# lisqzqng/GaVA-CLIP

Hardware: AMD Instinct MI355X
Metric: clips/sec (8-frame 224^2 ViT-B/16 VitaCLIP.forward) (higher is better)
Workload: dtype fp16; 1 GPU; c2: ViT-B/16, 8 frames, 224^2, batch 64/GPU, 3 classes; clips_per_gpu=64, global_batch=64, frames=8, classes=3, weights=random-init, parallelism=single GPU, text_tower=split-precision GEMMs (3 MFMA passes), fp32 softmax core

## Files before the change

gava_clip_amd/csrc/forward.hip:

```cpp
#include "common.h"
#include "internal.h"
#include <stdlib.h>
#include <mutex>

namespace {

struct SideStream {
  hipStream_t s = nullptr;
  hipEvent_t fork[64], join[64];
  bool ok = false, tried = false;
  bool get() {
    if (tried) return ok;
    tried = true;
    const char* e = getenv("GAVA_SIDE_STREAM");
    if (e && e[0] == '0') return false;
    int lo = 0, hi = 0;
    if (hipDeviceGetStreamPriorityRange(&lo, &hi) != hipSuccess) return false;
    if (hipStreamCreateWithPriority(&s, hipStreamNonBlocking, hi) != hipSuccess) return false;
    for (int i = 0; i < 64; ++i)
      if (hipEventCreateWithFlags(&fork[i], hipEventDisableTiming) != hipSuccess ||
          hipEventCreateWithFlags(&join[i], hipEventDisableTiming) != hipSuccess) return false;
    ok = true;
    return true;
  }
};

struct Fc1Probe {
  hipEvent_t ev[64][2];
  bool made = false;
  int on = 0;
  int n = 0;
  unsigned long long valid = 0;
  bool ensure() {
    if (made) return true;
    for (int i = 0; i < 64; ++i)
      for (int k = 0; k < 2; ++k)
        if (hipEventCreate(&ev[i][k]) != hipSuccess) return false;
    made = true;
    return true;
  }
};

constexpr int MAX_DEVICES = 64;
struct DeviceCtx {
  std::mutex mu;
  SideStream side;
  Fc1Probe probe;
};
DeviceCtx g_dev[MAX_DEVICES];
DeviceCtx& device_ctx() {
  int d = 0;
  if (hipGetDevice(&d) != hipSuccess || d < 0) d = 0;
  return g_dev[d % MAX_DEVICES];
}

struct Side {
  const SideStream& st; hipStream_t s; bool two;
  Side(SideStream& side, hipStream_t s, int layers) : st(side), s(s), two(side.get() && layers <= 64) {}
  gava_stream_t stream() const { return two ? (gava_stream_t)st.s : (gava_stream_t)s; }
  int fork(int i) const {
    return !two || (hipEventRecord(st.fork[i], s) == hipSuccess && hipStreamWaitEvent(st.s, st.fork[i], 0) == hipSuccess)
               ? GAVA_OK : GAVA_ELAUNCH;
  }
  int done(int i) const { return !two || hipEventRecord(st.join[i], st.s) == hipSuccess ? GAVA_OK : GAVA_ELAUNCH; }
  int join(int i) const { return !two || hipStreamWaitEvent(s, st.join[i], 0) == hipSuccess ? GAVA_OK : GAVA_ELAUNCH; }
  int cus(bool ln1_folded) const { return two ? (ln1_folded ? 32 : 8) : 0; }
};

struct Carver {
  char* base; size_t off, cap;
  Carver(void* b, size_t c) : base((char*)b), off(0), cap(c) {}
  void* take(size_t bytes) {
    const size_t a = (off + 255) & ~(size_t)255;
    off = a + bytes;
    return base ? (void*)(base + a) : nullptr;
  }
};

#define TRY(x)              \
  do {                      \
    const int _e = (x);     \
    if (_e != GAVA_OK) return _e; \
  } while (0)

int ln(const float* in, long in_stride, const int32_t* idx, const float* g, const float* b, void* o16, long o16s,
       float* o32, long o32s, int rows, int D, int prec, gava_stream_t s, int split = 0, const float* g2 = nullptr,
       const float* b2 = nullptr, void* ohi = nullptr, void* olo = nullptr, long ohls = 0) {
  gava_layernorm_args a{};
  a.gamma2 = g2; a.beta2 = b2;
  a.out_hi = ohi; a.out_lo = olo; a.out_hl_stride = ohls;
  a.in = in; a.in_stride = in_stride; a.in_row_index = idx; a.gamma = g; a.beta = b;
  a.out16 = o16; a.out16_stride = o16s; a.out32 = o32; a.out32_stride = o32s;
  a.rows = rows; a.D = D; a.prec = prec; a.split_out = split;
  return gava_layernorm(&a, s);
}

struct Fold {
  void* x16 = nullptr; long ld_x16 = 0; float* rowsum = nullptr; int reduced = 0;
  const float* stats = nullptr; const float* s = nullptr; const float* t = nullptr;
  const float* partials = nullptr;
  const void* r16 = nullptr; const void* rlo = nullptr; void* xlo = nullptr;
};

struct Lo8 {
  const void* A8 = nullptr; const void* W8 = nullptr; int exp = 0;
  void* out8 = nullptr; long ldo8 = 0; void* x8 = nullptr; long ldx8 = 0;
};

int gemm_x(int w_lo, const void* A, long lda, const void* W, long ldw, const float* bias, void* out, long ldo, int M, int N, int K,
           int epi, int prec, gava_stream_t s, const float* resid = nullptr, long ldr = 0, int scale_cols = 0,
           float scale = 1.f, int split_out = 0, void* aux_out = nullptr, const Fold* fold = nullptr, int cu_reserve = 0,
           const Lo8* l8 = nullptr) {
  gava_gemm_args a{};
  a.w_lo = w_lo ? 1 : 0;
  if (w_lo) ldw *= 2;
  if (l8) {
    if (l8->W8) {
      a.w_lo = 2; a.A8 = l8->A8; a.lda8 = 2 * lda; a.W8 = l8->W8; a.ldw8 = 2 * ldw; a.w8_exp = l8->exp;
    }
    a.out8 = l8->out8; a.ldo8 = l8->ldo8; a.x8_out = l8->x8; a.ld_x8 = l8->ldx8;
// ... 70 lines not shown
  w.XNC = c.take(BT * 3 * D * 2);
  w.QC = c.take(BT * D * 2);
  w.MIXC = c.take(BT * 3 * D * 2);
  w.HIDC = c.take(BT * 3 * F * 2);
  {
    const long per_slot = R * (D / 64) * 8, reduced = (R + 255) / 256 * 256 * 4 * 8 + 1024;
    w.RSUM = (float*)c.take(per_slot > reduced ? per_slot : reduced);
  }
  w.STATS = (float*)c.take((R + 255) / 256 * 256 * 8);
  w.Xn8 = m->w_lo == 2 ? c.take((size_t)R * 2 * D) : nullptr;
  w.HID8 = m->w_lo == 2 ? c.take((size_t)R * 2 * F) : nullptr;
  w.total = (c.off + 255) & ~(size_t)255;
  return w;
}

int check_vision(const gava_vision_model* m) {
  if (!m || !m->layer) return GAVA_EINVAL;
  if (m->B <= 0 || m->T_in <= 0 || m->T_model <= 0 || m->layers <= 0) return GAVA_EINVAL;
  if (m->size % m->P || m->D != m->H * 64 || m->D % 128 || m->F % 128 || m->E % 128) return GAVA_EINVAL;
  if (m->D > 1024) return GAVA_EINVAL;
  if (((long)m->B * m->T_in) % m->T_model) return GAVA_EINVAL;
  return GAVA_OK;
}

bool fused_stats(long R, int D) { return R >= 8192 && D % 256 == 0 && D <= 1024 && D >= 256; }

bool pair_stream(const gava_vision_model* m) {
  const long g = m->size / m->P, R = (long)m->B * m->T_in * (g * g + 1);
  const int D = m->D, F = m->F, WL = m->w_lo ? 2 : 1;
  bool pair = m->w_lo != 2 && m->layers >= 2 && fused_stats(R, D) &&
              gava::gemm_takes_pair((int)R, D, D, D, (long)WL * D) && gava::gemm_takes_pair((int)R, D, F, F, (long)WL * F);
  for (int i = 0; pair && i + 1 < m->layers; ++i) pair = m->layer[i].w_fc1_fold && m->layer[i + 1].w_qkv_fold;
  return pair;
}


struct VisionShape {
  int n, BT, R, D, F, E, H, G, Tm, pr, Kp, SR;
  long fs;
  explicit VisionShape(const gava_vision_model* m)
      : n((m->size / m->P) * (m->size / m->P)), BT(m->B * m->T_in), R(BT * (n + 1)), D(m->D), F(m->F), E(m->E), H(m->H),
        G(m->G), Tm(m->T_model), pr(m->prec), Kp(patch_k(m)), SR(G + 2 * BT), fs((long)(n + 1) * D) {}
};

int open_vision(const gava_vision_model* m, const float* x, const float* cls_x, const float* summary, void* workspace,
                size_t workspace_bytes, VisionWs* w) {
  TRY(check_vision(m));
  if ((!x && !m->clips) || !cls_x || !summary || !workspace) return GAVA_EINVAL;
  *w = carve_vision(m, workspace, workspace_bytes);
  return w->total > workspace_bytes ? GAVA_EWORKSPACE : GAVA_OK;
}

int embed(const gava_vision_model* m, const VisionShape& v, const float* x, int wl, float* out, void* scratch,
          gava_stream_t stream) {
  gava_gemm_args a{};
  a.W = m->w_patch; a.ldw = (wl ? 2 : 1) * v.Kp; a.bias = m->b_patch; a.w_lo = wl;
  a.out = out; a.ldo = v.D; a.M = v.BT * v.n; a.N = v.D; a.K = v.Kp; a.epilogue = GAVA_EPI_F32_PATCH; a.prec = v.pr;
  a.pos = m->pos_embed; a.time = m->time_embed; a.n_patches = v.n; a.T = m->T_in;
  TRY(patch_operand(m, x, scratch, stream, &a));
  TRY(gava_gemm(&a, stream));
  return gava::cls_embed(out, m->cls_token, m->pos_embed, m->time_embed, v.BT, m->T_in, v.D, v.fs, (hipStream_t)stream);
}

int prompt_path(const VisionShape& v, const gava_vision_layer& L, int wl, const VisionWs& w, const float* X, const void* hi,
                void* skv, gava_stream_t ss) {
  const int D = v.D, BT = v.BT, pr = v.pr;
  if (hi) {
    TRY(gemm_x(wl, hi, v.fs, L.w_cls, D, L.b_cls, w.CP, D, BT, D, D, GAVA_EPI_F32, pr, ss));
  } else {
    TRY(ln(X, v.fs, nullptr, nullptr, nullptr, w.CLS16, D, nullptr, 0, BT, D, pr, ss));
    TRY(gemm_x(wl, w.CLS16, D, L.w_cls, D, L.b_cls, w.CP, D, BT, D, D, GAVA_EPI_F32, pr, ss));
  }
  TRY(ln(w.CP, D, nullptr, L.sln_g, L.sln_b, w.CPn, D, nullptr, 0, BT, D, pr, ss));
  TRY(gemm_x(wl, w.CPn, D, L.w_sqkv, D, L.b_sqkv, w.SQKV, 3 * D, BT, 3 * D, D, GAVA_EPI_H16, pr, ss, nullptr, 0, D, 0.125f));
  {
    gava_attention_args a{};
    const unsigned short* q = (const unsigned short*)w.SQKV;
    a.q = q; a.k = q + D; a.v = q + 2 * D; a.ld_qkv = 3 * D; a.out = w.SMIX; a.ld_out = D;
    a.batch = BT / v.Tm; a.heads = v.H; a.n_q = v.Tm; a.n_kmain = v.Tm; a.prec = pr;
    TRY(gava_attention(&a, ss));
  }
  TRY(gemm_x(wl, w.SMIX, D, L.w_sout, D, L.b_sout, w.SUMM, D, BT, D, D, GAVA_EPI_F32, pr, ss, w.CP, D));
  TRY(gava::side_ln(L.global_prompts, L.local_prompts, w.CP, w.SUMM, L.ln1_g, L.ln1_b, w.SIDEn, v.G, v.Tm, BT, D, pr, (hipStream_t)ss));
  const unsigned short* wkv = (const unsigned short*)L.w_qkv + (long)D * (wl ? 2 : 1) * D;
  return gemm_x(wl, w.SIDEn, D, wkv, D, L.b_qkv + D, skv, 2 * D, v.SR, 2 * D, D, GAVA_EPI_H16, pr, ss);
}

struct FoldPlan {
  const VisionWs& w; int R, D; bool fused;
  FoldPlan(const VisionWs& w, int R, int D) : w(w), R(R), D(D), fused(fused_stats(R, D)) {}
  Fold produce() const {
    Fold p; p.x16 = w.Xn; p.ld_x16 = D; p.rowsum = w.RSUM; p.reduced = fused ? 1 : 0;
    return p;
  }
  Fold consume(const float* s, const float* t) const {
    Fold c; c.s = s; c.t = t;
    if (fused) c.partials = w.RSUM; else c.stats = w.STATS;
    return c;
  }
  int stats(gava_stream_t stream) const { return fused ? GAVA_OK : gava_row_stats(w.RSUM, D / 64, D, R, w.STATS, stream); }
};

int qkv_gemm(const VisionShape& v, const gava_vision_layer& L, int wl, bool kv_only, const FoldPlan& fp, const float* fold_s,
             const Lo8* lo, unsigned short* qkv, int resv, gava_stream_t stream) {
  const int D = v.D, c0 = kv_only ? D : 0;
  const unsigned short* W = (const unsigned short*)(fold_s ? L.w_qkv_fold : L.w_qkv) + (long)c0 * (wl ? 2 : 1) * D;
  const Fold c = fold_s ? fp.consume(fold_s + c0, L.qkv_fold_t + c0) : Fold{};
  return gemm_x(wl, fp.w.Xn, D, W, D, fold_s ? nullptr : L.b_qkv + c0, qkv + c0, 3 * D, v.R, 3 * D - c0, D, GAVA_EPI_H16, v.pr,
                stream, nullptr, 0, kv_only ? 0 : D, kv_only ? 1.f : 0.125f, 0, nullptr, fold_s ? &c : nullptr, resv, lo);
}

int cls_queries(const VisionShape& v, const gava_vision_layer& L, int wl, bool fold1, const float* X, const VisionWs& w, void* qc,
                gava_stream_t stream) {
  const int D = v.D;
  if (fold1) TRY(ln(X, v.fs, nullptr, L.ln1_g, L.ln1_b, w.XNC, D, nullptr, 0, v.BT, D, v.pr, stream));
  return gemm_x(wl, fold1 ? w.XNC : w.Xn, fold1 ? D : v.fs, L.w_qkv, D, L.b_qkv, qc, D, v.BT, D, D, GAVA_EPI_H16, v.pr, stream,
                nullptr, 0, D, 0.125f);
}

int frame_attention(const VisionShape& v, const unsigned short* qkv, const void* q, const void* skv, void* out, long ld_out,
                    int split_out, gava_stream_t stream) {
  const int D = v.D;
  const unsigned short* sk = (const unsigned short*)skv;
  gava_attention_args a{};
  a.q = q ? q : qkv;
  if (q) { a.ld_q = D; a.q_batch_rows = 1; }
  a.k = qkv + D; a.v = qkv + 2 * D; a.ld_qkv = 3 * D;
  a.side_k = sk; a.side_v = sk + D; a.ld_side = 2 * D;
  a.out = out; a.ld_out = ld_out; a.split_out = split_out;
  a.batch = v.BT; a.heads = v.H; a.n_q = q ? 1 : v.n + 1; a.n_kmain = v.n + 1;
  a.n_g = v.G; a.T = v.Tm; a.has_summary = 1; a.prec = v.pr;
  return gava_attention(&a, stream);
}

int head(const gava_vision_model* m, const VisionShape& v, const float* X, const VisionWs& w, float* cls_x, float* summary,
         gava_stream_t stream) {
  const int D = v.D, E = v.E, pr = v.pr;
  TRY(ln(X, v.fs, nullptr, m->lnpost_g, m->lnpost_b, w.CLSPOST, 3 * D, nullptr, 0, v.BT, D, pr, stream, 1));
  TRY(gemm(w.CLSPOST, 3 * D, m->w_proj, 3 * D, nullptr, w.PROJ, E, v.BT, E, 3 * D, GAVA_EPI_F32, pr, stream));
  TRY(gava::mean_rows(w.PROJ, cls_x, m->B, m->T_in, E, (hipStream_t)stream));
  return gava::mean_rows(w.SUMM, summary, v.BT / v.Tm, v.Tm, D, (hipStream_t)stream);
}

}

extern "C" int gava_vision_pair_stream(const gava_vision_model* m) {
  if (check_vision(m) != GAVA_OK) return 0;
  return pair_stream(m) ? 1 : 0;
}

#ifndef GAVA_ABI_HASH
#error "build with -DGAVA_ABI_HASH=<first 31 bits of sha256(include/gava_hip.h)> (python -m gava_clip_amd.build does)"
#endif
extern "C" int gava_abi_version(void) { return (int)(GAVA_ABI_HASH); }

extern "C" int gava_struct_sizes(size_t* out, int cap) {
  const size_t v[] = {sizeof(gava_gemm_args), sizeof(gava_layernorm_args), sizeof(gava_attention_args), sizeof(gava_attention_f32_args),
                      sizeof(gava_clip_desc), sizeof(gava_vision_layer), sizeof(gava_vision_layer8), sizeof(gava_vision_model),
                      sizeof(gava_text_layer), sizeof(gava_text_model), sizeof(gava_layernorm_bwd_args), sizeof(gava_attention_bwd_args),
                      sizeof(gava_vision_saved), sizeof(gava_preprocess_args), sizeof(gava_patchify_args),
                      sizeof(gava_preprocess_clips_args), sizeof(gava_view_scores_args)};
  const int n = (int)(sizeof(v) / sizeof(v[0]));
  for (int i = 0; out && i < n && i < cap; ++i) out[i] = v[i];
  return n;
}

extern "C" int gava_probe_fc1_enable(int on) {
  Fc1Probe& g_probe = device_ctx().probe;
  if (on < 0 || on > GAVA_PROBE_ATTN) return GAVA_EINVAL;
  g_probe.on = on; if (!on) g_probe.n = 0; return GAVA_OK;
}
extern "C" int gava_probe_fc1_read(float* ms, int cap) {
  Fc1Probe& g_probe = device_ctx().probe;
  const int n = g_probe.n;
  if (n <= 0 || !ms) return 0;
  if (hipEventSynchronize(g_probe.ev[n - 1][1]) != hipSuccess) return 0;
  for (int i = 0; i < n && i < cap; ++i) {
    ms[i] = -1.0f;
    if (((g_probe.valid >> i) & 1) && hipEventElapsedTime(&ms[i], g_probe.ev[i][0], g_probe.ev[i][1]) != hipSuccess) return 0;
  }
  return n;
}

extern "C" size_t gava_vision_workspace_bytes(const gava_vision_model* m) {
  if (check_vision(m) != GAVA_OK) return 0;
  return carve_vision(m, nullptr, 0).total;
}

extern "C" int gava_vision_forward(const gava_vision_model* m, const float* x, float* cls_x, float* summary,
                                   float* debug_cls, void* workspace, size_t workspace_bytes, gava_stream_t stream) {
  return gava_vision_forward_train(m, x, cls_x, summary, debug_cls, nullptr, workspace, workspace_bytes, stream);
}

extern "C" int gava_vision_forward_train(const gava_vision_model* m, const float* x, float* cls_x, float* summary,
                                         float* debug_cls, float* saved_x, void* workspace, size_t workspace_bytes,
                                         gava_stream_t stream) {
  VisionWs w;
  TRY(open_vision(m, x, cls_x, summary, workspace, workspace_bytes, &w));
  const int wl = m->w_lo ? 1 : 0;
  if (wl && saved_x) return GAVA_EINVAL;
  hipStream_t s = (hipStream_t)stream;
  DeviceCtx& dc = device_ctx();
  std::lock_guard<std::mutex> lock(dc.mu);
  Fc1Probe& g_probe = dc.probe;
  const VisionShape v(m);
  const int BT = v.BT, R = v.R, D = v.D, F = v.F, pr = v.pr;
  const long fs = v.fs;
  const bool l8 = m->w_lo == 2 && m->layer8 && pr == GAVA_PREC_F16 && D % 256 == 0 && F % 256 == 0;

  TRY(embed(m, v, x, wl, w.X, w.HID, stream));
  auto keep = [&](int slot) -> int {
    if (!saved_x) return GAVA_OK;
    return hipMemcpyAsync(saved_x + (size_t)slot * R * D, w.X, (size_t)R * D * sizeof(float), hipMemcpyDeviceToDevice, s) == hipSuccess
               ? GAVA_OK : GAVA_ELAUNCH;
  };
  TRY(keep(0));
#ifdef GAVA_ENABLE_ABLATE
  static const bool skip_attn = getenv("GAVA_DIAG_SKIP_ATTN") != nullptr, skip_stats = getenv("GAVA_DIAG_SKIP_STATS") != nullptr;
#else
  constexpr bool skip_attn = false, skip_stats = false;
#endif
  const bool pair = !saved_x && pair_stream(m);
  TRY(ln(w.X, D, nullptr, m->lnpre_g, m->lnpre_b, w.Xn, D, pair ? nullptr : w.X, D, R, D, pr, stream, 0, m->layer[0].ln1_g, m->layer[0].ln1_b,
         pair ? w.HID : nullptr, pair ? w.Xlo : nullptr, D));

  bool folded_in = false;
  const int probe = (g_probe.on && m->layers <= 64 && g_probe.ensure()) ? g_probe.on : 0;
  if (probe) { g_probe.n = 0; g_probe.valid = 0; }
  auto mark = [&](int which, int i, int k) -> int {
    if (probe != which) return GAVA_OK;
    if (hipEventRecord(g_probe.ev[i][k], s) != hipSuccess) return GAVA_ELAUNCH;
    if (k == 1) { g_probe.n = i + 1; g_probe.valid |= 1ull << i; }
    return GAVA_OK;
  };
  const Side side(dc.side, s, m->layers);
  const FoldPlan fp(w, R, D);
  Fold produce = fp.produce();
  if (pair) { produce.rlo = w.Xlo; produce.xlo = w.Xlo; }
  for (int i = 0; i < m->layers; ++i) {
    const gava_vision_layer& L = m->layer[i];
    TRY(keep(1 + i));
    TRY(side.fork(i));
    const void* hi_in = i == 0 ? w.HID : w.Xn;
    TRY(prompt_path(v, L, wl, w, w.X, pair ? hi_in : nullptr, w.SIDEKV, side.stream()));
    TRY(side.done(i));
    const int resv = side.cus(folded_in);
    const bool not_last = i + 1 < m->layers;
    const bool fold2 = !saved_x && not_last && L.w_fc1_fold && D % 64 == 0;
    const bool fold1 = folded_in;
    const bool fold1_next = !saved_x && not_last && m->layer[i + 1].w_qkv_fold && D % 64 == 0;
    if (!fold1 && i > 0) TRY(ln(w.X, D, nullptr, L.ln1_g, L.ln1_b, w.Xn, D, nullptr, 0, R, D, pr, stream));
    const gava_vision_layer8* L8 = l8 ? &m->layer8[i] : nullptr;
    const float* qkv_s = fold1 ? (L8 ? L8->qkv_fold_s8 : L.qkv_fold_s) : nullptr;
    if (not_last) {
      Lo8 lq; if (L8) { lq.A8 = w.Xn8; lq.W8 = L8->w_qkv_fold8; lq.exp = L8->qkv_fold_exp; }
      if (fold1) TRY(mark(GAVA_PROBE_QKV, i, 0));
      TRY(qkv_gemm(v, L, wl, false, fp, qkv_s, fold1 && L8 ? &lq : nullptr, (unsigned short*)w.QKV, resv, stream));
      if (fold1) TRY(mark(GAVA_PROBE_QKV, i, 1));
      TRY(side.join(i));
      TRY(mark(GAVA_PROBE_ATTN, i, 0));
      if (!skip_attn) TRY(frame_attention(v, (const unsigned short*)w.QKV, nullptr, w.SIDEKV, w.MIX, D, 0, stream));
      TRY(mark(GAVA_PROBE_ATTN, i, 1));
      TRY(mark(GAVA_PROBE_OUT, i, 0));
      if (fold2) {
        Lo8 po; if (L8) { po.x8 = w.Xn8; po.ldx8 = 2 * D; }
        if (pair) {
          produce.r16 = hi_in;
          TRY(gemm_x(wl, w.MIX, D, L.w_out, D, L.b_out, nullptr, 0, R, D, D, GAVA_EPI_F32, pr, stream, nullptr, D, 0, 1.f, 0, nullptr, &produce));
        } else
        TRY(gemm_x(wl, w.MIX, D, L.w_out, D, L.b_out, w.X, D, R, D, D, GAVA_EPI_F32, pr, stream, w.X, D, 0, 1.f, 0, nullptr, &produce, 0, L8 ? &po : nullptr));
        TRY(mark(GAVA_PROBE_OUT, i, 1));
        if (!skip_stats) TRY(fp.stats(stream));
        Fold c = fp.consume(L8 ? L8->fc1_fold_s8 : L.fc1_fold_s, L.fc1_fold_t);
        Lo8 lo; if (L8) { lo.A8 = w.Xn8; lo.W8 = L8->w_fc1_fold8; lo.exp = L8->fc1_fold_exp; lo.out8 = w.HID8; lo.ldo8 = 2 * F; }
        TRY(mark(GAVA_PROBE_FC1, i, 0));
        TRY(gemm_x(wl, w.Xn, D, L.w_fc1_fold, D, nullptr, w.HID, F, R, F, D, GAVA_EPI_H16_QGELU, pr, stream, nullptr, 0, 0, 1.f, 0, nullptr, &c, 0, L8 ? &lo : nullptr));
        TRY(mark(GAVA_PROBE_FC1, i, 1));
      } else {
        TRY(gemm_x(wl, w.MIX, D, L.w_out, D, L.b_out, w.X, D, R, D, D, GAVA_EPI_F32, pr, stream, w.X, D));
        TRY(mark(GAVA_PROBE_OUT, i, 1));
        TRY(ln(w.X, D, nullptr, L.ln2_g, L.ln2_b, w.Xn, D, nullptr, 0, R, D, pr, stream));
        TRY(mark(GAVA_PROBE_FC1, i, 0));
        TRY(gemm_x(wl, w.Xn, D, L.w_fc1, D, L.b_fc1, w.HID, F, R, F, D, GAVA_EPI_H16_QGELU, pr, stream));
        TRY(mark(GAVA_PROBE_FC1, i, 1));
      }
      TRY(mark(GAVA_PROBE_FC2, i, 0));
      Lo8 f2; const bool f2_8 = L8 && fold2;
      if (f2_8) { f2.A8 = w.HID8; f2.W8 = L8->w_fc28; f2.exp = L8->fc2_exp; }
      if (fold1_next) {
        if (L8) { f2.x8 = w.Xn8; f2.ldx8 = 2 * D; }
        if (pair) {
          produce.r16 = w.Xn;
          TRY(gemm_x(wl, w.HID, F, L.w_fc2, F, L.b_fc2, nullptr, 0, R, D, F, GAVA_EPI_F32, pr, stream, nullptr, D, 0, 1.f, 0, nullptr, &produce));
        } else
        TRY(gemm_x(wl, w.HID, F, L.w_fc2, F, L.b_fc2, w.X, D, R, D, F, GAVA_EPI_F32, pr, stream, w.X, D, 0, 1.f, 0, nullptr, &produce, 0, L8 ? &f2 : nullptr));
        TRY(mark(GAVA_PROBE_FC2, i, 1));
        if (!skip_stats) TRY(fp.stats(stream));
      } else {
        TRY(gemm_x(wl, w.HID, F, L.w_fc2, F, L.b_fc2, w.X, D, R, D, F, GAVA_EPI_F32, pr, stream, w.X, D, 0, 1.f, 0, nullptr, nullptr, 0, f2_8 ? &f2 : nullptr));
        TRY(mark(GAVA_PROBE_FC2, i, 1));
      }
      folded_in = fold1_next;
    } else {
      if (pair) TRY(gava::join_rows(w.Xn, w.Xlo, fs, w.X, fs, BT, D, pr, s));
      Lo8 lo; if (L8) { lo.A8 = w.Xn8; lo.W8 = (const char*)L8->w_qkv_fold8 + (size_t)D * 4 * D; lo.exp = L8->qkv_fold_exp; }
      TRY(qkv_gemm(v, L, wl, true, fp, qkv_s, fold1 && L8 ? &lo : nullptr, (unsigned short*)w.QKV, resv, stream));
      const int sp = (!saved_x && L.w_q_split && L.w_out_split && L.w_fc1_split && L.w_fc2_split) ? 1 : 0;
      const int S = sp ? 3 : 1;
      if (sp) {
        TRY(ln(w.X, fs, nullptr, L.ln1_g, L.ln1_b, w.XNC, 3 * D, nullptr, 0, BT, D, pr, stream, 1));
        TRY(gemm(w.XNC, 3 * D, L.w_q_split, 3 * D, L.b_qkv, w.QC, D, BT, D, 3 * D, GAVA_EPI_H16, pr, stream, nullptr, 0, D, 0.125f));
      } else {
        TRY(cls_queries(v, L, wl, fold1, w.X, w, w.QC, stream));
      }
      TRY(side.join(i));
      TRY(frame_attention(v, (const unsigned short*)w.QKV, w.QC, w.SIDEKV, w.MIXC, S * D, sp, stream));
      TRY(gemm_x(sp ? 0 : wl, w.MIXC, S * D, sp ? L.w_out_split : L.w_out, S * D, L.b_out, w.X, fs, BT, D, S * D, GAVA_EPI_F32, pr, stream, w.X, fs));
      TRY(ln(w.X, fs, nullptr, L.ln2_g, L.ln2_b, w.XNC, S * D, nullptr, 0, BT, D, pr, stream, sp));
      TRY(gemm_x(sp ? 0 : wl, w.XNC, S * D, sp ? L.w_fc1_split : L.w_fc1, S * D, L.b_fc1, w.HIDC, S * F, BT, F, S * D, GAVA_EPI_H16_QGELU, pr, stream, nullptr, 0, 0, 1.f, sp));
      TRY(gemm_x(sp ? 0 : wl, w.HIDC, S * F, sp ? L.w_fc2_split : L.w_fc2, S * F, L.b_fc2, w.X, fs, BT, D, S * F, GAVA_EPI_F32, pr, stream, w.X, fs));
    }
    if (debug_cls) {
      if (pair && not_last) TRY(gava::join_rows(w.Xn, w.Xlo, fs, debug_cls + (long)i * BT * D, D, BT, D, pr, s));
      else TRY(gava::copy_rows(w.X, fs, debug_cls + (long)i * BT * D, BT, D, s));
    }
  }

  TRY(keep(1 + m->layers));
  return head(m, v, w.X, w, cls_x, summary, stream);
}

extern "C" int gava_vision_forward_keep(const gava_vision_model* m, const float* x, float* cls_x, float* summary,
                                        const gava_vision_saved* sv, void* workspace, size_t workspace_bytes,
                                        gava_stream_t stream) {
  if (!m || m->w_lo || !sv || !sv->e0 || !sv->x || !sv->x1 || !sv->qkv || !sv->pre || !sv->sidekv) return GAVA_EINVAL;
  VisionWs w;
  TRY(open_vision(m, x, cls_x, summary, workspace, workspace_bytes, &w));
  DeviceCtx& dc = device_ctx();
  std::lock_guard<std::mutex> lock(dc.mu);
  const VisionShape v(m);
  const int BT = v.BT, R = v.R, D = v.D, F = v.F, pr = v.pr, SR = v.SR;
  const long fs = v.fs;
  const size_t RD = (size_t)R * D;
  TRY(embed(m, v, x, 0, sv->e0, w.HID, stream));
  const bool can_fold = D % 64 == 0 && m->layer[0].w_fc1_fold && m->layer[0].w_qkv_fold;
  const FoldPlan fp(w, R, D);
  const Fold produce = fp.produce();
  if (can_fold) TRY(ln(sv->e0, D, nullptr, m->lnpre_g, m->lnpre_b, w.Xn, D, sv->x, D, R, D, pr, stream, 0, m->layer[0].ln1_g, m->layer[0].ln1_b));
  else TRY(ln(sv->e0, D, nullptr, m->lnpre_g, m->lnpre_b, nullptr, 0, sv->x, D, R, D, pr, stream));
  bool folded_in = false;
  const Side side(dc.side, (hipStream_t)stream, m->layers);
  for (int i = 0; i < m->layers; ++i) {
    const gava_vision_layer& L = m->layer[i];
    float* Xin = sv->x + (size_t)i * RD;
    float* X1 = sv->x1 + (size_t)i * RD;
    float* Xout = sv->x + (size_t)(i + 1) * RD;
    unsigned short* QKV = (unsigned short*)sv->qkv + (size_t)i * R * 3 * D;
    unsigned short* PRE = (unsigned short*)sv->pre + (size_t)i * R * F;
    unsigned short* SKV = (unsigned short*)sv->sidekv + (size_t)i * SR * 2 * D;
    TRY(side.fork(i));
    TRY(prompt_path(v, L, 0, w, Xin, nullptr, SKV, side.stream()));
    TRY(side.done(i));
    const bool last_cls = i + 1 == m->layers && sv->last_q && sv->last_x1 && sv->last_pre;
    const bool fold1 = folded_in;
    const bool fold2 = can_fold && !last_cls && L.w_fc1_fold;
    const bool fold1_next = can_fold && i + 1 < m->layers && m->layer[i + 1].w_qkv_fold;
    const int resv = side.cus(fold1);
    if (!fold1 && !(i == 0 && can_fold)) TRY(ln(Xin, D, nullptr, L.ln1_g, L.ln1_b, w.Xn, D, nullptr, 0, R, D, pr, stream));
    const float* qkv_s = fold1 ? L.qkv_fold_s : nullptr;
    if (last_cls) {
      unsigned short* QC = (unsigned short*)sv->last_q;
      unsigned short* PREC = (unsigned short*)sv->last_pre;
      TRY(qkv_gemm(v, L, 0, true, fp, qkv_s, nullptr, QKV, resv, stream));
      TRY(cls_queries(v, L, 0, fold1, Xin, w, QC, stream));
      TRY(side.join(i));
      TRY(frame_attention(v, QKV, QC, SKV, w.MIXC, D, 0, stream));
      TRY(gemm(w.MIXC, D, L.w_out, D, L.b_out, sv->last_x1, D, BT, D, D, GAVA_EPI_F32, pr, stream, Xin, fs));
      TRY(ln(sv->last_x1, D, nullptr, L.ln2_g, L.ln2_b, w.XNC, D, nullptr, 0, BT, D, pr, stream));
      TRY(gemm(w.XNC, D, L.w_fc1, D, L.b_fc1, w.HIDC, F, BT, F, D, GAVA_EPI_H16_QGELU, pr, stream, nullptr, 0, 0, 1.f, 0, PREC));
      TRY(gemm(w.HIDC, F, L.w_fc2, F, L.b_fc2, Xout, fs, BT, D, F, GAVA_EPI_F32, pr, stream, sv->last_x1, D));
      continue;
    }
// ... 110 lines not shown
```

gava_clip_amd/csrc/internal.h:

```cpp
#pragma once
#include <hip/hip_runtime.h>
#include "../../include/gava_hip.h"
namespace gava {
int side_ln(const float* gp, const float* lp, const float* cp, const float* summ, const float* gamma,
            const float* beta, void* out, int G, int T, int BT, int D, int prec, hipStream_t s);
int cls_embed(float* X, const float* cls, const float* pos, const float* time, int BT, int T, int D,
              long frame_stride, hipStream_t s);
int mean_rows(const float* in, float* out, int B, int T, int D, hipStream_t s);
int copy_rows(const float* in, long in_stride, float* out, int rows, int D, hipStream_t s);
int join_rows(const void* hi, const void* lo, long in_stride, float* out, long out_stride, int rows, int D, int prec, hipStream_t s);
bool gemm_takes_pair(int M, int N, int K, long lda, long ldw);
bool gemm_patch_on_persistent(int M, int N, long lda, long ldw);
int text_embed(const float* emb, const float* pos, const float* ctx, const int* tok, float* X,
               int n_prompts, int L, int W, int n_ctx, hipStream_t s);
int train_head_forward(const float* video, const float* text, const int* offsets, const float* logit_scale, const float* logit_bias,
                       int B, int C, int P, int E, float* logits, float* text_features, float* video_norm, float* video_inv,
                       float* text_norm, float* text_inv, float* class_mean, hipStream_t s);
unsigned long long* debug_buffer();
bool stream_forced();

struct KeyRowSrc { bool is_main; long row; };
__device__ __forceinline__ KeyRowSrc key_row_src(int frame, int row, int n_kmain, int n_keys, int n_g, int T, int batch) {
  const int rowc = row < n_keys ? row : 0;
  const int sidx = rowc - n_kmain;
  const long sr = sidx < n_g ? sidx
                : sidx < n_g + T ? n_g + (long)(frame / T) * T + (sidx - n_g)
                                 : (long)n_g + batch + frame;
  const bool is_main = rowc < n_kmain;
  return {is_main, is_main ? (long)frame * n_kmain + rowc : sr};
}

struct AttnBwdMfmaParams {
  const unsigned short* q; const unsigned short* k; const unsigned short* v; long ld_qkv;
  long ld_q, ld_dq; int q_rows;
  const unsigned short* sk; const unsigned short* sv; long ld_side;
  const unsigned short* dout; long ld_dout;
  unsigned short* dq; unsigned short* dk; unsigned short* dv; long ld_dqkv;
  float* dsk; float* dsv; long ld_dside;
  float* stats;
  int batch, heads, n_q, n_kmain, n_g, T, has_summary, n_keys, q_pad;
  float q_scale;
};
int attention_bwd_mfma(const AttnBwdMfmaParams& p, int prec, int act_prec, int causal, hipStream_t s);
}
```

gava_clip_amd/csrc/rowops.hip:

```cpp
#include <cstdlib>
#include "common.h"
#include "internal.h"

namespace {

constexpr int MAXV = 4;

template <class P>
static __device__ __forceinline__ void store_h16x4(unsigned short* dst, float4 v) {
  *reinterpret_cast<uint2*>(dst) = pack4<P>(v.x, v.y, v.z, v.w);
}

static __device__ __forceinline__ void ln_row(float4 (&v)[MAXV], int nv_lane_count, int D,
                                              const bool (&act)[MAXV]) {
  float s = 0.f;
#pragma unroll
  for (int i = 0; i < MAXV; ++i)
    if (act[i]) s += (v[i].x + v[i].y) + (v[i].z + v[i].w);
  const float mean = wave_sum(s) / (float)D;
  float q = 0.f;
#pragma unroll
  for (int i = 0; i < MAXV; ++i)
    if (act[i]) {
      v[i].x -= mean; v[i].y -= mean; v[i].z -= mean; v[i].w -= mean;
// ... 104 lines not shown
};

template <class P>
__global__ __launch_bounds__(256) void side_ln_kernel(const SideParams p) {
  const int lane = threadIdx.x & 63;
  const int row = blockIdx.x * 4 + (threadIdx.x >> 6);
  if (row >= p.G + 2 * p.BT) return;
  float4 v[MAXV];
  bool act[MAXV];
#pragma unroll
  for (int i = 0; i < MAXV; ++i) {
    const int c = (lane + 64 * i) * 4;
    act[i] = c < p.D;
    if (!act[i]) continue;
    if (row < p.G) {
      v[i] = *reinterpret_cast<const float4*>(p.gp + (long)row * p.D + c);
    } else if (row < p.G + p.BT) {
      const int f = row - p.G;
      const float4 a = *reinterpret_cast<const float4*>(p.lp + (long)(f % p.T) * p.D + c);
      const float4 b = *reinterpret_cast<const float4*>(p.cp + (long)f * p.D + c);
      v[i] = make_float4(a.x + b.x, a.y + b.y, a.z + b.z, a.w + b.w);
    } else {
      v[i] = *reinterpret_cast<const float4*>(p.summ + (long)(row - p.G - p.BT) * p.D + c);
    }
  }
  ln_row(v, 0, p.D, act);
#pragma unroll
  for (int i = 0; i < MAXV; ++i)
    if (act[i]) {
      const int c = (lane + 64 * i) * 4;
      const float4 g = *reinterpret_cast<const float4*>(p.gamma + c);
      const float4 b = *reinterpret_cast<const float4*>(p.beta + c);
      store_h16x4<P>(p.out + (long)row * p.D + c,
                     make_float4(v[i].x * g.x + b.x, v[i].y * g.y + b.y, v[i].z * g.z + b.z, v[i].w * g.w + b.w));
    }
}

__global__ void cls_embed_kernel(float* X, const float* cls, const float* pos, const float* time,
                                 int BT, int T, int D, long frame_stride) {
  const long id = (long)blockIdx.x * blockDim.x + threadIdx.x;
  if (id >= (long)BT * D) return;
  const int c = (int)(id % D);
  const long f = id / D;
  X[f * frame_stride + c] = cls[c] + pos[c] + time[(f % T) * D + c];
}

__global__ void mean_rows_kernel(const float* in, float* out, int B, int T, int D) {
  const long id = (long)blockIdx.x * blockDim.x + threadIdx.x;
  if (id >= (long)B * D) return;
  const int c = (int)(id % D);
  const long b = id / D;
  float s = 0.f;
  for (int t = 0; t < T; ++t) s += in[(b * T + t) * D + c];
  out[id] = s / (float)T;
}

template <class P>
__global__ void join_rows_kernel(const unsigned short* hi, const unsigned short* lo, long in_stride, float* out, long out_stride,
                                 int rows, int D) {
  const long id = (long)blockIdx.x * blockDim.x + threadIdx.x;
  if (id >= (long)rows * D) return;
  const long r = id / D, c = id % D;
  out[r * out_stride + c] = P::up(hi[r * in_stride + c]) + PrecF16::up(lo[r * in_stride + c]);
}

__global__ void copy_rows_kernel(const float* in, long in_stride, float* out, int rows, int D) {
  const long id = (long)blockIdx.x * blockDim.x + threadIdx.x;
  if (id >= (long)rows * D) return;
  out[id] = in[(id / D) * in_stride + id % D];
}

__global__ void text_embed_kernel(const float* emb, const float* pos, const float* ctx, const int* tok,
                                  float* X, int n_prompts, int L, int W, int n_ctx) {
  const long id = (long)blockIdx.x * blockDim.x + threadIdx.x;
  if (id >= (long)n_prompts * L * W) return;
  const int c = (int)(id % W);
  const long row = id / W;
  const int l = (int)(row % L);
  const long n = row / L;
  float v;
  if (!tok) v = ctx[id];
  else if (l >= 1 && l <= n_ctx) v = ctx[(n * n_ctx + (l - 1)) * W + c];
  else v = emb[(long)tok[n * L + l] * W + c];
  X[id] = v + pos[(long)l * W + c];
}

template <class P>
__global__ void convert_kernel(const float* in, unsigned short* out, size_t n) {
  for (size_t i = (size_t)blockIdx.x * blockDim.x + threadIdx.x; i < n; i += (size_t)gridDim.x * blockDim.x)
    out[i] = P::cvt(in[i]);
}

__global__ void l2norm_rows_kernel(const float* in, float* out, int rows, int E, float* inv_out) {
  const int lane = threadIdx.x & 63;
  const int row = blockIdx.x * 4 + (threadIdx.x >> 6);
  if (row >= rows) return;
  float s = 0.f;
  for (int c = lane; c < E; c += 64) { const float v = in[(long)row * E + c]; s += v * v; }
  const float inv = 1.0f / sqrtf(wave_sum(s));
  for (int c = lane; c < E; c += 64) out[(long)row * E + c] = in[(long)row * E + c] * inv;
  if (inv_out && lane == 0) inv_out[row] = inv;
}

__global__ __launch_bounds__(64) void logits_mfma_kernel(const float* vn, const float* tn, const float* logit_scale,
                                                         const float* logit_bias, int B, int C, int E, float* logits) {
  const int lane = threadIdx.x;
// ... 200 lines not shown
extern "C" int gava_similarity_head(const float* video, const float* text, const float* logit_scale,
                                    const float* logit_bias, int B, int C, int n_kv, int E, float* logits,
                                    float* text_features, float* video_norm, gava_stream_t stream) {
  if (!video || !text || !logit_scale || !logits || !text_features || !video_norm) return GAVA_EINVAL;
  if (B <= 0 || C <= 0 || E <= 0 || n_kv <= 0 || E % 4) return GAVA_EINVAL;
  hipStream_t s = (hipStream_t)stream;
  hipLaunchKernelGGL(l2norm_rows_kernel, dim3((B + 3) / 4), dim3(256), 0, s, video, video_norm, B, E, (float*)nullptr);
  if (n_kv == 1) hipLaunchKernelGGL(l2norm_rows_kernel, dim3((C + 3) / 4), dim3(256), 0, s, text, text_features, C, E, (float*)nullptr);
  else hipLaunchKernelGGL(class_mean_kernel, dim3((C + 3) / 4), dim3(256), 0, s, text, text_features, C, n_kv, E,
                          (const int*)nullptr, 0, (float*)nullptr, (float*)nullptr);
  hipLaunchKernelGGL(logits_mfma_kernel, dim3(((B + 15) / 16) * ((C + 15) / 16)), dim3(64), 0, s, video_norm,
                     text_features, logit_scale, logit_bias, B, C, E, logits);
  hipLaunchKernelGGL(text_feature_kernel, dim3((C + 3) / 4), dim3(256), 0, s, text_features, text_features, C, 1, E);
  GAVA_CHECK_LAUNCH();
  return GAVA_OK;
}

static unsigned long long* g_debug_buffer = nullptr;
extern "C" int gava_debug_set_buffer(void* dev_u64) {
  g_debug_buffer = (unsigned long long*)dev_u64;
  return GAVA_OK;
}
namespace gava {
unsigned long long* debug_buffer() { return g_debug_buffer; }
}

namespace gava {

int side_ln(const float* gp, const float* lp, const float* cp, const float* summ, const float* gamma,
            const float* beta, void* out, int G, int T, int BT, int D, int prec, hipStream_t s) {
  SideParams p{gp, lp, cp, summ, gamma, beta, (unsigned short*)out, G, T, BT, D};
  const int rows = G + 2 * BT;
  if (prec == GAVA_PREC_F16) hipLaunchKernelGGL(side_ln_kernel<PrecF16>, dim3((rows + 3) / 4), dim3(256), 0, s, p);
  else hipLaunchKernelGGL(side_ln_kernel<PrecBF16>, dim3((rows + 3) / 4), dim3(256), 0, s, p);
  GAVA_CHECK_LAUNCH();
  return GAVA_OK;
}

int cls_embed(float* X, const float* cls, const float* pos, const float* time, int BT, int T, int D,
              long frame_stride, hipStream_t s) {
  const long n = (long)BT * D;
  hipLaunchKernelGGL(cls_embed_kernel, dim3((unsigned)((n + 255) / 256)), dim3(256), 0, s, X, cls, pos, time, BT, T, D, frame_stride);
  GAVA_CHECK_LAUNCH();
  return GAVA_OK;
}

int mean_rows(const float* in, float* out, int B, int T, int D, hipStream_t s) {
  const long n = (long)B * D;
  hipLaunchKernelGGL(mean_rows_kernel, dim3((unsigned)((n + 255) / 256)), dim3(256), 0, s, in, out, B, T, D);
  GAVA_CHECK_LAUNCH();
  return GAVA_OK;
}

int copy_rows(const float* in, long in_stride, float* out, int rows, int D, hipStream_t s) {
  const long n = (long)rows * D;
  hipLaunchKernelGGL(copy_rows_kernel, dim3((unsigned)((n + 255) / 256)), dim3(256), 0, s, in, in_stride, out, rows, D);
  GAVA_CHECK_LAUNCH();
  return GAVA_OK;
}

int join_rows(const void* hi, const void* lo, long in_stride, float* out, long out_stride, int rows, int D, int prec, hipStream_t s) {
  const long n = (long)rows * D;
  const dim3 grid((unsigned)((n + 255) / 256)), block(256);
  if (prec == GAVA_PREC_F16)
    hipLaunchKernelGGL(join_rows_kernel<PrecF16>, grid, block, 0, s, (const unsigned short*)hi, (const unsigned short*)lo, in_stride, out, out_stride, rows, D);
  else if (prec == GAVA_PREC_BF16)
    hipLaunchKernelGGL(join_rows_kernel<PrecBF16>, grid, block, 0, s, (const unsigned short*)hi, (const unsigned short*)lo, in_stride, out, out_stride, rows, D);
  else return GAVA_EINVAL;
  GAVA_CHECK_LAUNCH();
  return GAVA_OK;
}

int train_head_forward(const float* video, const float* text, const int* offsets, const float* logit_scale, const float* logit_bias,
                       int B, int C, int P, int E, float* logits, float* text_features, float* video_norm, float* video_inv,
                       float* text_norm, float* text_inv, float* class_mean, hipStream_t s) {
  hipLaunchKernelGGL(l2norm_rows_kernel, dim3((B + 3) / 4), dim3(256), 0, s, video, video_norm, B, E, video_inv);
  hipLaunchKernelGGL(class_mean_kernel, dim3((C + 3) / 4), dim3(256), 0, s, text, class_mean, C, 0, E, offsets, P, text_norm, text_inv);
  hipLaunchKernelGGL(logits_mfma_kernel, dim3(((B + 15) / 16) * ((C + 15) / 16)), dim3(64), 0, s, video_norm, class_mean,
                     logit_scale, logit_bias, B, C, E, logits);
  hipLaunchKernelGGL(text_feature_kernel, dim3((C + 3) / 4), dim3(256), 0, s, class_mean, text_features, C, 1, E);
  GAVA_CHECK_LAUNCH();
  return GAVA_OK;
}

int text_embed(const float* emb, const float* pos, const float* ctx, const int* tok, float* X,
               int n_prompts, int L, int W, int n_ctx, hipStream_t s) {
  const long n = (long)n_prompts * L * W;
  hipLaunchKernelGGL(text_embed_kernel, dim3((unsigned)((n + 255) / 256)), dim3(256), 0, s, emb, pos, ctx, tok, X, n_prompts, L, W, n_ctx);
  GAVA_CHECK_LAUNCH();
  return GAVA_OK;
}

}
```

Baseline: 3181 clips/s.

## Overlap serial front, last-layer query path and head means on side stream

Moves the CLS embedding, pre-LN and the first layer's prompt path onto the high-priority side stream so they run while the patch-embedding GEMM executes on the main stream. For the last layer, the row rejoin and CLS query projection also move onto the side stream. In the head, the two mean reductions are fused into one launch. This shortens the serial chain at both ends of the forward pass at the cost of more event synchronisation and an env-var controlled path.

Result: no change. 3173 clips/s (-0.2%).

```diff
diff --git a/gava_clip_amd/csrc/forward.hip b/gava_clip_amd/csrc/forward.hip
--- a/gava_clip_amd/csrc/forward.hip
+++ b/gava_clip_amd/csrc/forward.hip
@@ -1,6 +1,7 @@
 #include "common.h"
 #include "internal.h"
 #include <stdlib.h>
+#include <string.h>
 #include <mutex>
 
 namespace {
@@ -8,6 +9,7 @@
 struct SideStream {
   hipStream_t s = nullptr;
   hipEvent_t fork[64], join[64];
+  hipEvent_t front, cls;
   bool ok = false, tried = false;
   bool get() {
     if (tried) return ok;
@@ -20,6 +22,8 @@
     for (int i = 0; i < 64; ++i)
       if (hipEventCreateWithFlags(&fork[i], hipEventDisableTiming) != hipSuccess ||
           hipEventCreateWithFlags(&join[i], hipEventDisableTiming) != hipSuccess) return false;
+    if (hipEventCreateWithFlags(&front, hipEventDisableTiming) != hipSuccess ||
+        hipEventCreateWithFlags(&cls, hipEventDisableTiming) != hipSuccess) return false;
     ok = true;
     return true;
   }
@@ -64,8 +68,20 @@
   }
   int done(int i) const { return !two || hipEventRecord(st.join[i], st.s) == hipSuccess ? GAVA_OK : GAVA_ELAUNCH; }
   int join(int i) const { return !two || hipStreamWaitEvent(s, st.join[i], 0) == hipSuccess ? GAVA_OK : GAVA_ELAUNCH; }
+  int fork_front() const {
+    return hipEventRecord(st.front, s) == hipSuccess && hipStreamWaitEvent(st.s, st.front, 0) == hipSuccess ? GAVA_OK : GAVA_ELAUNCH;
+  }
+  int cls_done() const { return hipEventRecord(st.cls, st.s) == hipSuccess ? GAVA_OK : GAVA_ELAUNCH; }
+  int cls_wait() const { return hipStreamWaitEvent(s, st.cls, 0) == hipSuccess ? GAVA_OK : GAVA_ELAUNCH; }
   int cus(bool ln1_folded) const { return two ? (ln1_folded ? 32 : 8) : 0; }
 };
+
+enum { ENDS_FRONT = 1, ENDS_LAST = 2, ENDS_HEAD = 4 };
+int serial_ends() {
+  const char* e = getenv("GAVA_SERIAL_ENDS");
+  if (!e || !e[0] || e[0] == '1') return ENDS_FRONT | ENDS_LAST | ENDS_HEAD;
+  return (strstr(e, "front") ? ENDS_FRONT : 0) | (strstr(e, "last") ? ENDS_LAST : 0) | (strstr(e, "head") ? ENDS_HEAD : 0);
+}
 
 struct Carver {
   char* base; size_t off, cap;
@@ -242,20 +258,23 @@
 }
 
 int embed(const gava_vision_model* m, const VisionShape& v, const float* x, int wl, float* out, void* scratch,
-          gava_stream_t stream) {
+          gava_stream_t stream, bool cls_rows = true) {
   gava_gemm_args a{};
   a.W = m->w_patch; a.ldw = (wl ? 2 : 1) * v.Kp; a.bias = m->b_patch; a.w_lo = wl;
   a.out = out; a.ldo = v.D; a.M = v.BT * v.n; a.N = v.D; a.K = v.Kp; a.epilogue = GAVA_EPI_F32_PATCH; a.prec = v.pr;
   a.pos = m->pos_embed; a.time = m->time_embed; a.n_patches = v.n; a.T = m->T_in;
   TRY(patch_operand(m, x, scratch, stream, &a));
   TRY(gava_gemm(&a, stream));
+  if (!cls_rows) return GAVA_OK;
   return gava::cls_embed(out, m->cls_token, m->pos_embed, m->time_embed, v.BT, m->T_in, v.D, v.fs, (hipStream_t)stream);
 }
 
 int prompt_path(const VisionShape& v, const gava_vision_layer& L, int wl, const VisionWs& w, const float* X, const void* hi,
-                void* skv, gava_stream_t ss) {
+                void* skv, gava_stream_t ss, bool cls16_ready = false) {
   const int D = v.D, BT = v.BT, pr = v.pr;
-  if (hi) {
+  if (cls16_ready) {
+    TRY(gemm_x(wl, w.CLS16, D, L.w_cls, D, L.b_cls, w.CP, D, BT, D, D, GAVA_EPI_F32, pr, ss));
+  } else if (hi) {
     TRY(gemm_x(wl, hi, v.fs, L.w_cls, D, L.b_cls, w.CP, D, BT, D, D, GAVA_EPI_F32, pr, ss));
   } else {
     TRY(ln(X, v.fs, nullptr, nullptr, nullptr, w.CLS16, D, nullptr, 0, BT, D, pr, ss));
@@ -324,10 +343,11 @@
 }
 
 int head(const gava_vision_model* m, const VisionShape& v, const float* X, const VisionWs& w, float* cls_x, float* summary,
-         gava_stream_t stream) {
+         gava_stream_t stream, bool one_mean = false) {
   const int D = v.D, E = v.E, pr = v.pr;
   TRY(ln(X, v.fs, nullptr, m->lnpost_g, m->lnpost_b, w.CLSPOST, 3 * D, nullptr, 0, v.BT, D, pr, stream, 1));
   TRY(gemm(w.CLSPOST, 3 * D, m->w_proj, 3 * D, nullptr, w.PROJ, E, v.BT, E, 3 * D, GAVA_EPI_F32, pr, stream));
+  if (one_mean) return gava::mean_rows2(w.PROJ, cls_x, m->B, m->T_in, E, w.SUMM, summary, v.BT / v.Tm, v.Tm, D, (hipStream_t)stream);
   TRY(gava::mean_rows(w.PROJ, cls_x, m->B, m->T_in, E, (hipStream_t)stream));
   return gava::mean_rows(w.SUMM, summary, v.BT / v.Tm, v.Tm, D, (hipStream_t)stream);
 }
@@ -398,7 +418,20 @@
   const long fs = v.fs;
   const bool l8 = m->w_lo == 2 && m->layer8 && pr == GAVA_PREC_F16 && D % 256 == 0 && F % 256 == 0;
 
-  TRY(embed(m, v, x, wl, w.X, w.HID, stream));
+  const Side side(dc.side, s, m->layers);
+  const int ends = serial_ends();
+  const bool early = (ends & ENDS_FRONT) && side.two;
+  if (early) {
+    gava_stream_t ss = side.stream();
+    TRY(side.fork_front());
+    TRY(gava::cls_embed(w.X, m->cls_token, m->pos_embed, m->time_embed, BT, m->T_in, D, fs, (hipStream_t)ss));
+    TRY(ln(w.X, fs, nullptr, m->lnpre_g, m->lnpre_b, w.CLS16, D, nullptr, 0, BT, D, pr, ss));
+    TRY(side.cls_done());
+    TRY(prompt_path(v, m->layer[0], wl, w, w.X, nullptr, w.SIDEKV, ss, true));
+    TRY(side.done(0));
+  }
+  TRY(embed(m, v, x, wl, w.X, w.HID, stream, !early));
+  if (early) TRY(side.cls_wait());
   auto keep = [&](int slot) -> int {
     if (!saved_x) return GAVA_OK;
     return hipMemcpyAsync(saved_x + (size_t)slot * R * D, w.X, (size_t)R * D * sizeof(float), hipMemcpyDeviceToDevice, s) == hipSuccess
@@ -423,21 +456,36 @@
     if (k == 1) { g_probe.n = i + 1; g_probe.valid |= 1ull << i; }
     return GAVA_OK;
   };
-  const Side side(dc.side, s, m->layers);
   const FoldPlan fp(w, R, D);
   Fold produce = fp.produce();
   if (pair) { produce.rlo = w.Xlo; produce.xlo = w.Xlo; }
   for (int i = 0; i < m->layers; ++i) {
     const gava_vision_layer& L = m->layer[i];
+    const bool not_last = i + 1 < m->layers;
+    const bool fold1 = folded_in;
+    const int sp = (!saved_x && L.w_q_split && L.w_out_split && L.w_fc1_split && L.w_fc2_split) ? 1 : 0;
+    auto rejoin = [&](gava_stream_t qs) -> int {
+      return pair ? gava::join_rows(w.Xn, w.Xlo, fs, w.X, fs, BT, D, pr, (hipStream_t)qs) : GAVA_OK;
+    };
+    auto queries = [&](gava_stream_t qs) -> int {
+      if (!sp) return cls_queries(v, L, wl, fold1, w.X, w, w.QC, qs);
+      TRY(ln(w.X, fs, nullptr, L.ln1_g, L.ln1_b, w.XNC, 3 * D, nullptr, 0, BT, D, pr, qs, 1));
+      return gemm(w.XNC, 3 * D, L.w_q_split, 3 * D, L.b_qkv, w.QC, D, BT, D, 3 * D, GAVA_EPI_H16, pr, qs, nullptr, 0, D, 0.125f);
+    };
+    const bool last_on_side = (ends & ENDS_LAST) && side.two && !not_last && i > 0 && (fold1 || sp);
     TRY(keep(1 + i));
-    TRY(side.fork(i));
     const void* hi_in = i == 0 ? w.HID : w.Xn;
-    TRY(prompt_path(v, L, wl, w, w.X, pair ? hi_in : nullptr, w.SIDEKV, side.stream()));
-    TRY(side.done(i));
+    if (!(early && i == 0)) {
+      TRY(side.fork(i));
+      TRY(prompt_path(v, L, wl, w, w.X, pair ? hi_in : nullptr, w.SIDEKV, side.stream()));
+      if (last_on_side) {
+        TRY(rejoin(side.stream()));
+        TRY(queries(side.stream()));
+      }
+      TRY(side.done(i));
+    }
     const int resv = side.cus(folded_in);
-    const bool not_last = i + 1 < m->layers;
     const bool fold2 = !saved_x && not_last && L.w_fc1_fold && D % 64 == 0;
-    const bool fold1 = folded_in;
     const bool fold1_next = !saved_x && not_last && m->layer[i + 1].w_qkv_fold && D % 64 == 0;
     if (!fold1 && i > 0) TRY(ln(w.X, D, nullptr, L.ln1_g, L.ln1_b, w.Xn, D, nullptr, 0, R, D, pr, stream));
     const gava_vision_layer8* L8 = l8 ? &m->layer8[i] : nullptr;
@@ -492,17 +540,11 @@
       }
       folded_in = fold1_next;
     } else {
-      if (pair) TRY(gava::join_rows(w.Xn, w.Xlo, fs, w.X, fs, BT, D, pr, s));
+      if (!last_on_side) TRY(rejoin(stream));
       Lo8 lo; if (L8) { lo.A8 = w.Xn8; lo.W8 = (const char*)L8->w_qkv_fold8 + (size_t)D * 4 * D; lo.exp = L8->qkv_fold_exp; }
       TRY(qkv_gemm(v, L, wl, true, fp, qkv_s, fold1 && L8 ? &lo : nullptr, (unsigned short*)w.QKV, resv, stream));
-      const int sp = (!saved_x && L.w_q_split && L.w_out_split && L.w_fc1_split && L.w_fc2_split) ? 1 : 0;
       const int S = sp ? 3 : 1;
-      if (sp) {
-        TRY(ln(w.X, fs, nullptr, L.ln1_g, L.ln1_b, w.XNC, 3 * D, nullptr, 0, BT, D, pr, stream, 1));
-        TRY(gemm(w.XNC, 3 * D, L.w_q_split, 3 * D, L.b_qkv, w.QC, D, BT, D, 3 * D, GAVA_EPI_H16, pr, stream, nullptr, 0, D, 0.125f));
-      } else {
-        TRY(cls_queries(v, L, wl, fold1, w.X, w, w.QC, stream));
-      }
+      if (!last_on_side) TRY(queries(stream));
       TRY(side.join(i));
       TRY(frame_attention(v, (const unsigned short*)w.QKV, w.QC, w.SIDEKV, w.MIXC, S * D, sp, stream));
       TRY(gemm_x(sp ? 0 : wl, w.MIXC, S * D, sp ? L.w_out_split : L.w_out, S * D, L.b_out, w.X, fs, BT, D, S * D, GAVA_EPI_F32, pr, stream, w.X, fs));
@@ -517,7 +559,7 @@
   }
 
   TRY(keep(1 + m->layers));
-  return head(m, v, w.X, w, cls_x, summary, stream);
+  return head(m, v, w.X, w, cls_x, summary, stream, (ends & ENDS_HEAD) != 0);
 }
 
 extern "C" int gava_vision_forward_keep(const gava_vision_model* m, const float* x, float* cls_x, float* summary,
diff --git a/gava_clip_amd/csrc/internal.h b/gava_clip_amd/csrc/internal.h
--- a/gava_clip_amd/csrc/internal.h
+++ b/gava_clip_amd/csrc/internal.h
@@ -7,6 +7,8 @@
 int cls_embed(float* X, const float* cls, const float* pos, const float* time, int BT, int T, int D,
               long frame_stride, hipStream_t s);
 int mean_rows(const float* in, float* out, int B, int T, int D, hipStream_t s);
+int mean_rows2(const float* in0, float* out0, int B0, int T0, int D0, const float* in1, float* out1, int B1, int T1, int D1,
+               hipStream_t s);
 int copy_rows(const float* in, long in_stride, float* out, int rows, int D, hipStream_t s);
 int join_rows(const void* hi, const void* lo, long in_stride, float* out, long out_stride, int rows, int D, int prec, hipStream_t s);
 bool gemm_takes_pair(int M, int N, int K, long lda, long ldw);
diff --git a/gava_clip_amd/csrc/rowops.hip b/gava_clip_amd/csrc/rowops.hip
--- a/gava_clip_amd/csrc/rowops.hip
+++ b/gava_clip_amd/csrc/rowops.hip
@@ -180,6 +180,23 @@
   const long b = id / D;
   float s = 0.f;
   for (int t = 0; t < T; ++t) s += in[(b * T + t) * D + c];
+  out[id] = s / (float)T;
+}
+
+struct MeanSeg { const float* in; float* out; int B, T, D; };
+__global__ void mean_rows2_kernel(const MeanSeg a, const MeanSeg b) {
+  long id = (long)blockIdx.x * blockDim.x + threadIdx.x;
+  const long na = (long)a.B * a.D;
+  const bool first = id < na;
+  const float* in = first ? a.in : b.in;
+  float* out = first ? a.out : b.out;
+  const int B = first ? a.B : b.B, T = first ? a.T : b.T, D = first ? a.D : b.D;
+  if (!first) id -= na;
+  if (id >= (long)B * D) return;
+  const int c = (int)(id % D);
+  const long r = id / D;
+  float s = 0.f;
+  for (int t = 0; t < T; ++t) s += in[(r * T + t) * D + c];
   out[id] = s / (float)T;
 }
 
@@ -486,6 +503,15 @@
   return GAVA_OK;
 }
 
+int mean_rows2(const float* in0, float* out0, int B0, int T0, int D0, const float* in1, float* out1, int B1, int T1, int D1,
+               hipStream_t s) {
+  const long n = (long)B0 * D0 + (long)B1 * D1;
+  const MeanSeg a{in0, out0, B0, T0, D0}, b{in1, out1, B1, T1, D1};
+  hipLaunchKernelGGL(mean_rows2_kernel, dim3((unsigned)((n + 255) / 256)), dim3(256), 0, s, a, b);
+  GAVA_CHECK_LAUNCH();
+  return GAVA_OK;
+}
+
 int copy_rows(const float* in, long in_stride, float* out, int rows, int D, hipStream_t s) {
   const long n = (long)rows * D;
   hipLaunchKernelGGL(copy_rows_kernel, dim3((unsigned)((n + 255) / 256)), dim3(256), 0, s, in, in_stride, out, rows, D);
```
